# PPWangyc/video-spike

Hardware: AMD Instinct MI355X
Metric: clips/sec (16-frame 224x224) train step (higher is better)
Workload: dtype bf16; 1 GPU; C2 ViT-Tiny/16 16x224x224 -> 128 neurons, encoder+head fwd+bwd+AdamW; model=vmae_tiny, global_batch=128, clips_per_gpu=128, seq_len=1568, parallelism=dp1

## Files before the change

include/vspike.h:

```cpp
#ifndef VSPIKE_H
#define VSPIKE_H

#include <stddef.h>
#include <stdint.h>

#ifdef __cplusplus
extern "C" {
#endif

#define VS_OK 0
#define VS_EINVAL (-1)

#define VS_F32 0
#define VS_BF16 1
#define VS_U8 2
#define VS_F64 4
#define VS_FP8 3

int vs_version(void);
const char* vs_build_id(void);
const char* vs_last_error(void);
int vs_device_arch(char* buf, int n);
int vs_struct_size(int which);

// ... 308 lines not shown
#define VS_PATH_GEMM_FULLK    7
#define VS_PATH_GEMM_RING     8
#define VS_PATH_GEMM_TILE     9
#define VS_PATH_GEMM_F32     10
#define VS_PATH_GEMM_LN_FWD  11
#define VS_PATH_GEMM_LN_BWD  12
#define VS_PATH_ATTN_FWD     13
#define VS_PATH_ATTN_BWD     14
#define VS_PATH_ATTN_F32     15
#define VS_PATH_PATCH_FUSED  16
#define VS_PATH_DW_GROUPED   17
#define VS_PATH_MLP_FWD      18
#define VS_PATH_MLP_BWD      19
#define VS_PATH_GEMM_FP8     20
#define VS_PATH_PATCH_DW     21
#define VS_PATH_CONV_IGEMM   22
#define VS_PATH_CONV_DW      23
#define VS_PATH_GEMM_G256    24
#define VS_PATH_GEMM_DW256   25
#define VS_PATH_TOKEN_POOL   26
#define VS_PATH_CLS_EMBED    27
#define VS_PATH_EMBED_HEAD   28
#define VS_PATH_INFO_NCE     29
#define VS_PATH_COUNT        30
int vs_dispatch_counts(int64_t* out, int n);
int vs_dispatch_reset(void);
#define VS_LN_KERNELS 9
int vs_ln_dispatch_counts(int64_t* out, int n);
#define VS_RRR_PATH_WIDE   0
#define VS_RRR_PATH_SMOOTH 1
#define VS_RRR_PATH_COUNT  2
int vs_rrr_dispatch_counts(int64_t* out, int n);
int vs_g256_scratch_free(void);

#define VS_KNOB_DW_OLD       0
#define VS_KNOB_NO_SKINNY    1
#define VS_KNOB_NO_SLAB      2
#define VS_KNOB_NO_BIG       3
#define VS_KNOB_NO_WRES      4
#define VS_KNOB_WRES_GBWD    5
#define VS_KNOB_NO_WSLAB     6
#define VS_KNOB_WSLAB        7
#define VS_KNOB_WSLAB_G      8
#define VS_KNOB_PANEL        9
#define VS_KNOB_NO_PANEL    10
#define VS_KNOB_PANEL_GRID  11
#define VS_KNOB_NO_FULLK    12
#define VS_KNOB_NO_RING     13
#define VS_KNOB_NO_LNF_FUSE 14
#define VS_KNOB_NO_LN_FUSE  15
#define VS_KNOB_DW_BM       16
#define VS_KNOB_DW_BN       17
#define VS_KNOB_DW_SPLITS   18
#define VS_KNOB_DW_STAGES   19
#define VS_KNOB_LN_BLOCKS   20
#define VS_KNOB_DH_F32      21
#define VS_KNOB_NO_PATCH_FUSED 22
#define VS_KNOB_NO_DW_GROUP 23
#define VS_KNOB_ATTN_VARIANT 24
#define VS_KNOB_SLAB_WV     25
#define VS_KNOB_WRES_WV     26
#define VS_KNOB_WRES_DBG    27
#define VS_KNOB_G256        28
#define VS_KNOB_G256_GRID   29
#define VS_KNOB_G256_DBG    30
#define VS_KNOB_NO_DW256    31
#define VS_KNOB_G256_STAGGER 32
#define VS_KNOB_CONV_DW128  33
#define VS_KNOB_CONV_MFMA   34
#define VS_KNOB_DW256_ALL   36
#define VS_KNOB_LN_FWD_BLOCKS 37
#define VS_KNOB_G256_A3     35
#define VS_KNOB_COUNT       40
int vs_knob_get(int knob);
int vs_knob_set(int knob, int value);
int vs_knob_default(int knob);
int vs_debug_knobs(void);

#ifdef __cplusplus
}
#endif
#endif
```

video-spike_amd/csrc/gemm.hip:

```cpp
#include <cstdlib>

#include "common.h"
#include "gemm_common.h"
#include "gemm_dw.h"

namespace vs {

template <int BM, int BN, int TM, int TN, uint32_t EF, int PARTS = 1>
__device__ __forceinline__ void store_tile(const EpiParams& e, float* lds, const f32x4 (&acc)[TM][TN], int64_t m0,
                                           int64_t n0, int split) {
  static_assert(PARTS == 1 || (PARTS == 2 && BM / 2 == BM / 2 / 16 * 16), "row halves");
  const bool first_split = split == 0;
  const uint32_t F = epi_flags<EF>(e);
  constexpr int LDT = BN + 4;
  constexpr int WM = BM / 2, WN = BN / 2, RB = BM / PARTS;
  const int tid = threadIdx.x, lane = tid & 63, wid = tid >> 6, wr = wid >> 1, wc = wid & 1;
  constexpr int CPR = BN / 8;
  constexpr int RPP = 256 / CPR;
  const int cg = tid % CPR;
  const int64_t n = n0 + cg * 8;
  const bool vec = e.vec_ok && n + 8 <= e.N;
  float bias8[8];
  if ((F & VS_EPI_BIAS) && vec && !(F & VS_EPI_ATOMIC) && !e.part) ld8(e.bias, n, 0, bias8);
#pragma unroll
  for (int part = 0; part < PARTS; ++part) {
    const int64_t mp = m0 + part * RB;
    __syncthreads();
    if (PARTS == 1 || wr == part) {
#pragma unroll
      for (int i = 0; i < TM; ++i)
#pragma unroll
        for (int j = 0; j < TN; ++j)
// ... 517 lines not shown
  VS_GMARK(4);
#ifdef VS_STAMP
  if ((threadIdx.x & 63) == 0) {
    const int w_ = blockIdx.x * 4 + (threadIdx.x >> 6);
    if (w_ < 8192) {
      g_gstamp[8 * w_ + 5] = __builtin_amdgcn_s_getreg((31 << 11) | 4);
      g_gstamp[8 * w_ + 6] = __builtin_amdgcn_s_memrealtime();
    }
  }
#endif
}

struct LnBwdParams {
  const float* x;
  int64_t ldx;
  const float* mean;
  const float* rstd;
  const float* gamma;
  const float* dres;
  int64_t ldr;
  float* dx;
  int64_t lddx;
  bf16_t* dx_lp;
  float* part;
  const float* beta;
  float eps;
  bf16_t* h;
  int64_t ldh;
  float* mean_out;
  float* rstd_out;
};

template <int NT, bool BKC, uint32_t EF, bool LNB = false, bool LNF = false, int WV = 4>
__global__ __launch_bounds__(64 * WV, 2) __attribute__((amdgpu_waves_per_eu(WV / 2, WV / 2))) void gemm_bf16_slab_kernel(const bf16_t* __restrict__ A, int64_t lda,
                                                                const bf16_t* __restrict__ B, int64_t ldb, int64_t K,
                                                                EpiParams e, LnBwdParams ln) {
  constexpr int RT = 16 * WV, NTH = 64 * WV, PR = NTH / 16;
  using OA = OperandBf16<RT, true>;
  using OB = OperandBf16<64, BKC>;
  constexpr int N = 64 * NT, TM = 2, TN = NT * 2, WN = N / 2;
  constexpr int STAGE = OA::BYTES + NT * OB::BYTES;
  constexpr int LDT = N + 4;
  static_assert(64 * LDT * 4 <= 2 * STAGE, "epilogue staging (64 rows at a time) fits the ring");
  static_assert(WV == 4 || WV == 8, "4 or 8 waves");
  __shared__ __attribute__((aligned(16))) char smem[2 * STAGE];

  const int tid = threadIdx.x, lane = tid & 63, wid = tid >> 6, wr = wid >> 1, wc = wid & 1;
  const int64_t G = gridDim.x;
  const int64_t r_begin = (int64_t)blockIdx.x * e.M / G, r_end = ((int64_t)blockIdx.x + 1) * e.M / G;
  const int nk = (int)(K / 64);
  const int gl = tid & 15, rsub = tid >> 4;
  float4 pg[NT], pb[NT];
#pragma unroll
  for (int j = 0; j < NT; ++j) {
    pg[j] = make_float4(0.f, 0.f, 0.f, 0.f);
    pb[j] = make_float4(0.f, 0.f, 0.f, 0.f);
  }

  for (int64_t m0 = r_begin; m0 < r_end; m0 += RT) {
    const int64_t m_end = m0 + RT < r_end ? m0 + RT : r_end;
    f32x4 acc[TM][TN];
#pragma unroll
    for (int i = 0; i < TM; ++i)
#pragma unroll
      for (int j = 0; j < TN; ++j) acc[i][j] = f32x4{0.f, 0.f, 0.f, 0.f};
    auto issue = [&](int t, char* st) {
      const int64_t k0 = (int64_t)t * 64;
// ... 219 lines not shown
  }
  if constexpr (LNB) {
    float* red = (float*)smem;
    __syncthreads();
#pragma unroll
    for (int j = 0; j < NT; ++j) {
#define VS_RED(V)                               \
  {                                             \
    _Pragma("unroll") for (int o = 16; o < 64; o <<= 1) { \
      V.x += __shfl_xor(V.x, o, 64);            \
      V.y += __shfl_xor(V.y, o, 64);            \
      V.z += __shfl_xor(V.z, o, 64);            \
      V.w += __shfl_xor(V.w, o, 64);            \
    }                                           \
  }
      VS_RED(pg[j]) VS_RED(pb[j])
#undef VS_RED
      if (lane < 16) {
        *(float4*)&red[(0 * WV + wid) * N + 4 * (gl + 16 * j)] = pg[j];
        *(float4*)&red[(1 * WV + wid) * N + 4 * (gl + 16 * j)] = pb[j];
      }
    }
    __syncthreads();
    for (int c = tid; c < N; c += NTH) {
      float a = (red[0 * N + c] + red[1 * N + c]) + (red[2 * N + c] + red[3 * N + c]);
      float b = (red[WV * N + c] + red[(WV + 1) * N + c]) + (red[(WV + 2) * N + c] + red[(WV + 3) * N + c]);
      if constexpr (WV == 8) {
        a += (red[4 * N + c] + red[5 * N + c]) + (red[6 * N + c] + red[7 * N + c]);
        b += (red[12 * N + c] + red[13 * N + c]) + (red[14 * N + c] + red[15 * N + c]);
      }
      ln.part[(int64_t)blockIdx.x * 2 * N + c] = a;
      ln.part[(int64_t)blockIdx.x * 2 * N + N + c] = b;
    }
  }
}

struct PatchGeo {
  int F, C, H, W;
  int n_tok, HpWp, Wp;
};

template <int NT, bool COLS>
__global__ __launch_bounds__(256, 2) void patch_embed_fwd_kernel(const float* __restrict__ px, PatchGeo g,
                                                                 const bf16_t* __restrict__ B, int64_t K,
                                                                 EpiParams e, bf16_t* __restrict__ cols) {
  using OA = OperandBf16<64, true>;
  using OB = OperandBf16<64, true>;
  constexpr int N = 64 * NT, TM = 2, TN = NT * 2, WN = N / 2, NR = 3;
  constexpr int STAGE = OA::BYTES + NT * OB::BYTES;
  constexpr int LDT = N + 4;
  static_assert(64 * LDT * 4 <= 2 * STAGE, "epilogue staging fits the ring");
  __shared__ __attribute__((aligned(16))) char smem[2 * STAGE];

  const int tid = threadIdx.x, lane = tid & 63, wid = tid >> 6, wr = wid >> 1, wc = wid & 1;
  const int64_t G = gridDim.x;
  const int64_t r_begin = (int64_t)blockIdx.x * e.M / G, r_end = ((int64_t)blockIdx.x + 1) * e.M / G;
  const int nk = (int)(K / 64);
  const int ii = (tid >> 2) & 3, jq = tid & 3;
  const int64_t plane = (int64_t)g.H * g.W;

  for (int64_t m0 = r_begin; m0 < r_end; m0 += 64) {
    const int64_t m_end = m0 + 64 < r_end ? m0 + 64 : r_end;
    int64_t base[4];
#pragma unroll
    for (int s = 0; s < 4; ++s) {
      int64_t m = m0 + (tid >> 4) + 16 * s;
// ... 1338 lines not shown
}

template <int BM, int BN, uint32_t EF>
static void launch_bf16_ring_ef(const vs_gemm_desc* d, unsigned nblk, const GridMap& g, const EpiParams& e,
                                hipStream_t s) {
  const bf16_t* a = (const bf16_t*)d->a;
  const bf16_t* b = (const bf16_t*)d->b;
  if (d->a_kcontig && d->b_kcontig)
    hipLaunchKernelGGL((gemm_bf16_ring_kernel<BM, BN, true, true, EF>), dim3(nblk), dim3(256), 0, s, a, d->lda, b, d->ldb, d->K, g, e);
  else if (d->a_kcontig)
    hipLaunchKernelGGL((gemm_bf16_ring_kernel<BM, BN, true, false, EF>), dim3(nblk), dim3(256), 0, s, a, d->lda, b, d->ldb, d->K, g, e);
  else if (d->b_kcontig)
    hipLaunchKernelGGL((gemm_bf16_ring_kernel<BM, BN, false, true, EF>), dim3(nblk), dim3(256), 0, s, a, d->lda, b, d->ldb, d->K, g, e);
  else
    hipLaunchKernelGGL((gemm_bf16_ring_kernel<BM, BN, false, false, EF>), dim3(nblk), dim3(256), 0, s, a, d->lda, b, d->ldb, d->K, g, e);
}

template <int KT, uint32_t EF>
static void launch_bf16_panel_ef(const vs_gemm_desc* d, unsigned grid, int64_t items, const EpiParams& e,
                                 hipStream_t s) {
  const bf16_t* a = (const bf16_t*)d->a;
  const bf16_t* b = (const bf16_t*)d->b;
  if (d->b_kcontig)
    hipLaunchKernelGGL((gemm_bf16_panel_kernel<KT, true, EF>), dim3(grid), dim3(256), 0, s, a, d->lda, b, d->ldb, items, e);
  else
    hipLaunchKernelGGL((gemm_bf16_panel_kernel<KT, false, EF>), dim3(grid), dim3(256), 0, s, a, d->lda, b, d->ldb, items, e);
}

static inline bool slab_wide(int64_t M, int64_t K, unsigned grid) {
  const int f = knob(VS_KNOB_SLAB_WV);
  if (f == 4 || f == 8) return f == 8;
  return M / (int64_t)grid >= 256 && K >= 384;
}
template <int NT, uint32_t EF, bool LNB = false, bool LNF = false>
static void launch_bf16_slab_ef(const vs_gemm_desc* d, unsigned grid, const EpiParams& e, hipStream_t s,
                                const LnBwdParams& ln = LnBwdParams{}) {
  const bf16_t* a = (const bf16_t*)d->a;
  const bf16_t* b = (const bf16_t*)d->b;
  if (slab_wide(d->M, d->K, grid)) {
    if (d->b_kcontig)
      hipLaunchKernelGGL((gemm_bf16_slab_kernel<NT, true, EF, LNB, LNF, 8>), dim3(grid), dim3(512), 0, s, a, d->lda, b,
                         d->ldb, d->K, e, ln);
    else
      hipLaunchKernelGGL((gemm_bf16_slab_kernel<NT, false, EF, LNB, LNF, 8>), dim3(grid), dim3(512), 0, s, a, d->lda, b,
                         d->ldb, d->K, e, ln);
    return;
  }
  if (d->b_kcontig)
    hipLaunchKernelGGL((gemm_bf16_slab_kernel<NT, true, EF, LNB, LNF>), dim3(grid), dim3(256), 0, s, a, d->lda, b,
                       d->ldb, d->K, e, ln);
  else
    hipLaunchKernelGGL((gemm_bf16_slab_kernel<NT, false, EF, LNB, LNF>), dim3(grid), dim3(256), 0, s, a, d->lda, b,
                       d->ldb, d->K, e, ln);
}
template <int NT>
static void launch_bf16_slab(const vs_gemm_desc* d, unsigned grid, const EpiParams& e, hipStream_t s) {
  switch (e.flags) {
    case 0: launch_bf16_slab_ef<NT, 0u>(d, grid, e, s); break;
    case VS_EPI_BIAS: launch_bf16_slab_ef<NT, (uint32_t)VS_EPI_BIAS>(d, grid, e, s); break;
    case VS_EPI_BIAS | VS_EPI_POS:
      launch_bf16_slab_ef<NT, (uint32_t)(VS_EPI_BIAS | VS_EPI_POS)>(d, grid, e, s);
      break;
    default: launch_bf16_slab_ef<NT, (uint32_t)(VS_EPI_BIAS | VS_EPI_RESIDUAL)>(d, grid, e, s); break;
  }
}

template <int KT, uint32_t EF>
static void launch_bf16_wslab_ef(const vs_gemm_desc* d, unsigned grid, const EpiParams& e, hipStream_t s) {
  const bf16_t* a = (const bf16_t*)d->a;
  const bf16_t* b = (const bf16_t*)d->b;
  if (d->b_kcontig)
// ... 70 lines not shown
template <bool BKC, bool P8>
static int g256_no_scratch_all() {
  int ok = 1;
#define CHK_(EF)                                                                                    \
  {                                                                                                 \
    hipFuncAttributes fa{};                                                                          \
    if (hipFuncGetAttributes(&fa, (const void*)gemm_bf16_g256_kernel<BKC, P8, EF>) != hipSuccess || \
        fa.localSizeBytes != 0)                                                                     \
      ok = 0;                                                                                       \
  }
  CHK_(0u) CHK_((uint32_t)VS_EPI_BIAS) CHK_((uint32_t)(VS_EPI_BIAS | VS_EPI_RESIDUAL))
  CHK_((uint32_t)(VS_EPI_BIAS | VS_EPI_GELU)) CHK_((uint32_t)VS_EPI_GELU_BWD)
  CHK_((uint32_t)(VS_EPI_BIAS | VS_EPI_GELU | VS_EPI_GELU_GRAD)) CHK_((uint32_t)VS_EPI_MUL_AUX)
#undef CHK_
  return ok;
}

#define VS_EPI_SWITCH(F, CALL)                                                             \
  switch (F) {                                                                             \
    case 0: CALL(0u); break;                                                               \
    case VS_EPI_BIAS: CALL((uint32_t)VS_EPI_BIAS); break;                                  \
    case VS_EPI_BIAS | VS_EPI_RESIDUAL: CALL((uint32_t)(VS_EPI_BIAS | VS_EPI_RESIDUAL)); break; \
    case VS_EPI_BIAS | VS_EPI_GELU: CALL((uint32_t)(VS_EPI_BIAS | VS_EPI_GELU)); break;    \
    case VS_EPI_GELU_BWD: CALL((uint32_t)VS_EPI_GELU_BWD); break;                          \
    case VS_EPI_BIAS | VS_EPI_GELU | VS_EPI_GELU_GRAD:                                     \
      CALL((uint32_t)(VS_EPI_BIAS | VS_EPI_GELU | VS_EPI_GELU_GRAD)); break;               \
    case VS_EPI_MUL_AUX: CALL((uint32_t)VS_EPI_MUL_AUX); break;                            \
    default: CALL(kEpiRuntime); break;                                                     \
  }

extern "C" int vs_g256_scratch_free(void) {
  return g256_no_scratch_all<true, true>() & g256_no_scratch_all<false, true>() & g256_no_scratch_all<false, false>();
}

static void launch_bf16_g256(const vs_gemm_desc* d, const G256Map& g, unsigned grid, const EpiParams& e,
                             hipStream_t s) {
#define L_(EF) launch_bf16_g256_ef<EF>(d, g, grid, e, s)
  VS_EPI_SWITCH(e.flags, L_)
#undef L_
}

static void launch_bf16_big(const vs_gemm_desc* d, unsigned nblk, const GridMap& g, const EpiParams& e, hipStream_t s) {
#define L_(EF) launch_bf16_big_ef<EF>(d, nblk, g, e, s)
  VS_EPI_SWITCH(e.flags, L_)
#undef L_
}

template <int BM, int BN>
static void launch_bf16(const vs_gemm_desc* d, unsigned nblk, const GridMap& g, const EpiParams& e, hipStream_t s) {
#define L_(EF) launch_bf16_ef<BM, BN, EF>(d, nblk, g, e, s)
  VS_EPI_SWITCH(e.flags, L_)
#undef L_
}

template <int BM, int BN>
static void launch_bf16_ring(const vs_gemm_desc* d, unsigned nblk, const GridMap& g, const EpiParams& e, hipStream_t s) {
#define L_(EF) launch_bf16_ring_ef<BM, BN, EF>(d, nblk, g, e, s)
  VS_EPI_SWITCH(e.flags, L_)
#undef L_
}

template <int KT>
static void launch_bf16_panel(const vs_gemm_desc* d, unsigned grid, int64_t items, const EpiParams& e, hipStream_t s) {
#define L_(EF) launch_bf16_panel_ef<KT, EF>(d, grid, items, e, s)
  VS_EPI_SWITCH(e.flags, L_)
#undef L_
// ... 619 lines not shown
```

video-spike_amd/csrc/runtime.hip:

```cpp
#include <atomic>
#include <cstdlib>
#include <mutex>
#include <string.h>
#include <vector>

#include "common.h"

#ifndef VS_BUILD_ID
#define VS_BUILD_ID "unknown"
#endif

namespace vs {

static thread_local char g_err[512] = "";
thread_local int g_timer_tag = -1;

void set_error(const char* msg) {
  strncpy(g_err, msg, sizeof(g_err) - 1);
  g_err[sizeof(g_err) - 1] = 0;
}

struct KnobDef {
  const char* env;
  int dflt;
};
static const KnobDef kKnobs[VS_KNOB_COUNT] = {
    {"VSPIKE_DW_OLD", 0},      {"VSPIKE_NO_SKINNY", 0},    {"VSPIKE_NO_SLAB", 0},      {"VSPIKE_NO_BIG", 0},
    {"VSPIKE_NO_WRES", 0},     {"VSPIKE_WRES_GBWD", 0},    {"VSPIKE_NO_WSLAB", 0},     {"VSPIKE_WSLAB", 0},
    {"VSPIKE_WSLAB_G", 512},   {"VSPIKE_PANEL", 0},        {"VSPIKE_NO_PANEL", 0},     {"VSPIKE_PANEL_GRID", 512},
    {"VSPIKE_NO_FULLK", 0},    {"VSPIKE_NO_RING", 0},      {"VSPIKE_NO_LNF_FUSE", 0},  {"VSPIKE_NO_LN_FUSE", 0},
    {"VSPIKE_DW_BM", 0},       {"VSPIKE_DW_BN", 0},        {"VSPIKE_DW_SPLITS", 0},    {"VSPIKE_DW_STAGES", 0},
    {"VSPIKE_LN_BLOCKS", 0},   {"VSPIKE_DH_F32", 0},       {"VSPIKE_NO_PATCH_FUSED", 0}, {"VSPIKE_NO_DW_GROUP", 0},
    {"VSPIKE_ATTN_VARIANT", 0}, {"VSPIKE_SLAB_WV", 0}, {"VSPIKE_WRES_WV", 0}, {"VSPIKE_WRES_DBG", 0}, {"VSPIKE_G256", 0}, {"VSPIKE_G256_GRID", 0}, {"VSPIKE_G256_DBG", 0}, {"VSPIKE_NO_DW256", 0}, {"VSPIKE_G256_STAGGER", 0}, {"VSPIKE_CONV_DW128", 0},
    {"VSPIKE_CONV_MFMA", 0}, {"VSPIKE_G256_A3", 0}, {"VSPIKE_DW256_ALL", 0}, {"VSPIKE_LN_FWD_BLOCKS", 0},
    {nullptr, 0}};
static std::atomic<int> g_knob[VS_KNOB_COUNT];
static std::once_flag g_knob_once;
static void knob_init() {
  for (int i = 0; i < VS_KNOB_COUNT; ++i) {
    int v = kKnobs[i].dflt;
    if (kKnobs[i].env) {
      const char* e = getenv(kKnobs[i].env);
      if (e && e[0]) v = (int)strtol(e, nullptr, 0);
    }
    g_knob[i].store(v, std::memory_order_relaxed);
  }
}
int knob(int id) {
  std::call_once(g_knob_once, knob_init);
  return g_knob[id].load(std::memory_order_relaxed);
}

static std::atomic<int64_t> g_dispatch[VS_PATH_COUNT];
void count_path(int id) { g_dispatch[id].fetch_add(1, std::memory_order_relaxed); }
static std::atomic<int64_t> g_rrr_dispatch[VS_RRR_PATH_COUNT];
void count_rrr(int id) { g_rrr_dispatch[id].fetch_add(1, std::memory_order_relaxed); }
static std::atomic<int64_t> g_ln_dispatch[2 * VS_LN_KERNELS];
void count_ln(int kernel, bool bwd) {
  g_ln_dispatch[(bwd ? VS_LN_KERNELS : 0) + kernel].fetch_add(1, std::memory_order_relaxed);
}

struct TimerState {
  std::mutex mu;
  unsigned mask = 0;
  std::vector<hipEvent_t> pool;
  std::vector<std::pair<hipEvent_t, hipEvent_t>> pairs[VS_TIMER_COUNT];
  double bytes[VS_TIMER_COUNT] = {};
  hipEvent_t get() {
// ... 139 lines not shown
```

video-spike_amd/vspike/_lib.py:

```python
from __future__ import annotations

import ctypes
import os

import torch

from .build import LIB_PATH

VS_F32, VS_BF16, VS_U8, VS_FP8, VS_F64 = 0, 1, 2, 3, 4
EPI_BIAS, EPI_GELU, EPI_RELU, EPI_RESIDUAL, EPI_POS = 0x1, 0x2, 0x4, 0x8, 0x10
EPI_GELU_BWD, EPI_RELU_BWD, EPI_ATOMIC, EPI_ACCUM = 0x20, 0x40, 0x80, 0x100
EPI_GELU_GRAD, EPI_MUL_AUX = 0x200, 0x400
BWD_DEFER_JOIN = 0x1
BWD_DEFER_LAST = 0x2
BWD_FUSE_LN = 0x4
TIMER_ATTN_FWD, TIMER_ATTN_BWD, TIMER_GEMM, TIMER_GEMM_DW, TIMER_LN_FWD, TIMER_LN_BWD, TIMER_ADAMW, TIMER_MISC = range(8)
TIMER_NAMES = ("attn_fwd", "attn_bwd", "gemm", "gemm_dw", "ln_fwd", "ln_bwd", "adamw", "misc",
               "fwd_qkv", "fwd_proj", "fwd_fc1", "fwd_fc2", "dx_fc2", "dx_fc1", "dx_proj", "dx_qkv",
               "dw_fc2", "dw_fc1", "dw_proj", "dw_qkv",
               "fwd_mlp", "dx_mlp",
               "fp8_quant",
               "conv_fwd", "conv_dx", "conv_dw", "bn")

PATH_NAMES = ("gemm_dw", "gemm_skinny", "gemm_slab", "gemm_big", "gemm_wres", "gemm_wslab", "gemm_panel",
              "gemm_fullk", "gemm_ring", "gemm_tile", "gemm_f32", "gemm_ln_fwd", "gemm_ln_bwd", "attn_fwd",
              "attn_bwd", "attn_f32", "patch_fused", "dw_grouped", "mlp_fwd", "mlp_bwd", "gemm_fp8", "patch_dw",
              "conv_igemm", "conv_dw", "gemm_g256", "gemm_dw256", "token_pool")
PATH_COUNT = 27
CONTRAST_PATH_NAMES = ("cls_embed", "embed_head", "info_nce")
EXTRA_PATH_NAMES = CONTRAST_PATH_NAMES
KNOB_NAMES = ("dw_old", "no_skinny", "no_slab", "no_big", "no_wres", "wres_gbwd", "no_wslab", "wslab", "wslab_g",
              "panel", "no_panel", "panel_grid", "no_fullk", "no_ring", "no_lnf_fuse", "no_ln_fuse", "dw_bm", "dw_bn",
              "dw_splits", "dw_stages", "ln_blocks", "dh_f32", "no_patch_fused", "no_dw_group", "attn_variant", "slab_wv", "wres_wv", "wres_dbg",
              "g256", "g256_grid", "g256_dbg", "no_dw256", "g256_stagger", "conv_dw128", "conv_mfma", "g256_a3", "dw256_all", "ln_fwd_blocks")
KNOB_COUNT = 40

c_i32, c_i64, c_u32, c_f32, c_p, c_sz = (ctypes.c_int32, ctypes.c_int64, ctypes.c_uint32, ctypes.c_float,
                                         ctypes.c_void_p, ctypes.c_size_t)
c_f64 = ctypes.c_double


class VsError(RuntimeError):
    pass


class GemmDesc(ctypes.Structure):
    _fields_ = [("dtype", c_i32), ("out_dtype", c_i32), ("a_kcontig", c_i32), ("b_kcontig", c_i32),
                ("M", c_i64), ("N", c_i64), ("K", c_i64),
                ("a", c_p), ("lda", c_i64), ("b", c_p), ("ldb", c_i64), ("c", c_p), ("ldc", c_i64),
                ("epilogue", c_u32), ("alpha", c_f32), ("bias", c_p),
                ("residual", c_p), ("ld_residual", c_i64), ("pos", c_p), ("pos_rows", c_i64),
                ("aux_in", c_p), ("ld_aux_in", c_i64), ("aux_out", c_p), ("ld_aux_out", c_i64),
                ("split_k", c_i32), ("reserved", c_i32), ("a_rowsum", c_p), ("workspace", c_p),
                ("workspace_bytes", c_i64)]


class Conv3dDesc(ctypes.Structure):
    _fields_ = [("N", c_i64), ("Di", c_i64), ("Hi", c_i64), ("Wi", c_i64), ("Ci", c_i64),
                ("Do", c_i64), ("Ho", c_i64), ("Wo", c_i64), ("Co", c_i64),
                ("kd", c_i32), ("kh", c_i32), ("kw", c_i32), ("sd", c_i32), ("sh", c_i32), ("sw", c_i32),
                ("pd", c_i32), ("ph", c_i32), ("pw", c_i32), ("reserved", c_i32)]


class VitLayer(ctypes.Structure):
    _fields_ = [("dtype", c_i32), ("heads", c_i32), ("batch", c_i64), ("tokens", c_i64), ("hidden", c_i64),
                ("mlp", c_i64), ("ln_eps", c_f32), ("attn_scale", c_f32),
                ("ln1_g", c_p), ("ln1_b", c_p), ("ln2_g", c_p), ("ln2_b", c_p),
                ("w_qkv", c_p), ("b_qkv", c_p), ("w_proj", c_p), ("b_proj", c_p),
                ("w_fc1", c_p), ("b_fc1", c_p), ("w_fc2", c_p), ("b_fc2", c_p),
                ("x_in", c_p), ("h1", c_p), ("mean1", c_p), ("rstd1", c_p), ("qkv", c_p), ("attn_o", c_p),
                ("lse", c_p), ("y", c_p), ("h2", c_p), ("mean2", c_p), ("rstd2", c_p), ("a_pre", c_p),
                ("a_act", c_p), ("x_out", c_p), ("fp8_ws", c_p), ("fp8_ws_bytes", c_i64),
                ("next_ln_g", c_p), ("next_ln_b", c_p), ("next_h1", c_p), ("next_mean1", c_p), ("next_rstd1", c_p),
                ("ln1_ready", c_i32), ("reserved7", c_i32)]


class VitLayerGrad(ctypes.Structure):
    _fields_ = [("ln1_g", c_p), ("ln1_b", c_p), ("ln2_g", c_p), ("ln2_b", c_p),
                ("w_qkv", c_p), ("b_qkv", c_p), ("w_proj", c_p), ("b_proj", c_p),
                ("w_fc1", c_p), ("b_fc1", c_p), ("w_fc2", c_p), ("b_fc2", c_p),
                ("dx_out", c_p), ("dx_out_lp", c_p), ("dx_in", c_p), ("dx_in_lp", c_p),
                ("d_a", c_p), ("d_h", c_p), ("dy", c_p), ("dy_lp", c_p), ("d_o", c_p), ("d_qkv", c_p),
                ("attn_ws", c_p), ("ln_ws", c_p), ("gemm_ws", c_p), ("gemm_ws_bytes", c_i64),
                ("flags", c_i32), ("reserved", c_i32), ("chain", c_p)]


PROTOTYPES = {
    "vs_version": (ctypes.c_int, []),
    "vs_build_id": (ctypes.c_char_p, []),
    "vs_dispatch_counts": (ctypes.c_int, [ctypes.POINTER(c_i64), ctypes.c_int]),
    "vs_dispatch_reset": (ctypes.c_int, []),
    "vs_ln_dispatch_counts": (ctypes.c_int, [ctypes.POINTER(c_i64), ctypes.c_int]),
    "vs_g256_scratch_free": (ctypes.c_int, []),
    "vs_knob_get": (ctypes.c_int, [ctypes.c_int]),
    "vs_knob_set": (ctypes.c_int, [ctypes.c_int, ctypes.c_int]),
    "vs_knob_default": (ctypes.c_int, [ctypes.c_int]),
    "vs_debug_knobs": (ctypes.c_int, []),
    "vs_mse_loss": (ctypes.c_int, [c_i64, c_p, c_p, c_p, c_p, c_f32, c_p, c_p]),
    "vs_comm_unique_id": (ctypes.c_int, [c_p]),
    "vs_comm_init": (ctypes.c_int, [ctypes.POINTER(c_p), c_p, c_i32, c_i32]),
    "vs_comm_allreduce_bucket": (ctypes.c_int, [c_p, c_p, c_i64, c_i32, c_p]),
    "vs_comm_finalize": (ctypes.c_int, [c_p]),
    "vs_mse_loss_bwd": (ctypes.c_int, [c_i64, c_p, c_p, c_p, c_p, c_p]),
    "vs_last_error": (ctypes.c_char_p, []),
    "vs_device_arch": (ctypes.c_int, [ctypes.c_char_p, ctypes.c_int]),
    "vs_struct_size": (ctypes.c_int, [ctypes.c_int]),
    "vs_gemm": (ctypes.c_int, [ctypes.POINTER(GemmDesc), c_p]),
    "vs_layernorm_fwd": (ctypes.c_int, [c_i32, c_i64, c_i64, c_p, c_i64, c_p, c_p, c_f32, c_p, c_i64, c_p, c_p,
                                        c_p]),
    "vs_layernorm_bwd_workspace_bytes": (c_sz, [c_i64, c_i64]),
    "vs_gemm_splitk_workspace_bytes": (c_sz, [c_i32, c_i64, c_i64, c_i64]),
    "vs_video_preprocess": (ctypes.c_int, [c_i32, c_i64, c_i64, c_i64, c_i64, c_p, ctypes.POINTER(c_i32), c_i32,
                                           c_i64, ctypes.POINTER(c_f32), ctypes.POINTER(c_f32), c_p, c_p]),
    "vs_layernorm_bwd": (ctypes.c_int, [c_i64, c_i64, c_p, c_i64, c_p, c_i64, c_p, c_p, c_p, c_p, c_i64, c_p,
                                        c_i64, c_p, c_p, c_p, c_p, c_p]),
    "vs_layernorm_bwd_dt": (ctypes.c_int, [ctypes.c_int32, c_i64, c_i64, c_p, c_i64, c_p, c_i64, c_p, c_p, c_p, c_p, c_i64, c_p,
                                        c_i64, c_p, c_p, c_p, c_p, c_p]),
    "vs_gemm_ln_fwd": (ctypes.c_int, [ctypes.POINTER(GemmDesc), c_p, c_p, ctypes.c_float, c_p, c_i64, c_p, c_p, c_p]),
    "vs_gemm_ln_bwd": (ctypes.c_int, [ctypes.POINTER(GemmDesc), c_p, c_i64, c_p, c_p, c_p, c_p, c_i64, c_p, c_i64,
                                      c_p, c_p, c_p, c_p, c_p]),
    "vs_mlp_fused_ok": (ctypes.c_int, [c_i64, c_i64, c_i64]),
    "vs_mlp_fwd_ln": (ctypes.c_int, [c_i64, c_i64, c_i64, c_p, c_i64, c_p, c_p, c_p, c_p, c_p, c_i64, c_p, c_i64,
                                     c_p, c_p, c_f32, c_p, c_i64, c_p, c_p, c_p]),
    "vs_quant_mxfp8": (ctypes.c_int, [c_i32, c_i64, c_i64, c_p, c_i64, c_p, c_i64, c_p, c_i64, c_p]),
    "vs_gemm_mxfp8": (ctypes.c_int, [ctypes.POINTER(GemmDesc), c_p, c_i64, c_p, c_i64, c_p]),
    "vs_mlp_fwd": (ctypes.c_int, [c_i64, c_i64, c_i64, c_p, c_i64, c_p, c_p, c_p, c_p, c_p, c_i64, c_p, c_i64, c_p]),
# ... 233 lines not shown
```

Baseline: 4183 clips/sec.

## Add persistent triple-buffered slab GEMM kernel with fused LayerNorm backward

Adds a persistent 512-thread slab GEMM kernel with fused LayerNorm backward. It keeps three LDS stages and prefetches the next slab's first K tiles while the current slab's LN-backward epilogue runs, so slab boundaries no longer drain the load pipeline. The kernel is only used when a new knob is set to 1 (default 0) and K/64 is a multiple of 3, with grid size defaulting to the CU count. Separately, the existing slab kernel's waves-per-EU hint is fixed at 2 instead of WV/2, which changes register allocation and occupancy for the 8-wave variant on the default path. Occupancy and launch-count query helpers are also exported.

```diff
diff --git a/include/vspike.h b/include/vspike.h
--- a/include/vspike.h
+++ b/include/vspike.h
@@ -364,6 +364,9 @@
 #define VS_RRR_PATH_COUNT  2
 int vs_rrr_dispatch_counts(int64_t* out, int n);
 int vs_g256_scratch_free(void);
+int vs_slab_occupancy(int nt, int bkc, int lnb, int wv, int pipe);
+int vs_slab_pipe_grid(int slabs);
+int64_t vs_slab_pipe_launches(void);
 
 #define VS_KNOB_DW_OLD       0
 #define VS_KNOB_NO_SKINNY    1
@@ -403,6 +406,8 @@
 #define VS_KNOB_DW256_ALL   36
 #define VS_KNOB_LN_FWD_BLOCKS 37
 #define VS_KNOB_G256_A3     35
+#define VS_KNOB_SLAB_PIPE   38
+#define VS_KNOB_SLAB_PIPE_GRID 39
 #define VS_KNOB_COUNT       40
 int vs_knob_get(int knob);
 int vs_knob_set(int knob, int value);
diff --git a/video-spike_amd/csrc/gemm.hip b/video-spike_amd/csrc/gemm.hip
--- a/video-spike_amd/csrc/gemm.hip
+++ b/video-spike_amd/csrc/gemm.hip
@@ -1,3 +1,4 @@
+#include <atomic>
 #include <cstdlib>
 
 #include "common.h"
@@ -581,7 +582,7 @@
 };
 
 template <int NT, bool BKC, uint32_t EF, bool LNB = false, bool LNF = false, int WV = 4>
-__global__ __launch_bounds__(64 * WV, 2) __attribute__((amdgpu_waves_per_eu(WV / 2, WV / 2))) void gemm_bf16_slab_kernel(const bf16_t* __restrict__ A, int64_t lda,
+__global__ __launch_bounds__(64 * WV, 2) __attribute__((amdgpu_waves_per_eu(2, 2))) void gemm_bf16_slab_kernel(const bf16_t* __restrict__ A, int64_t lda,
                                                                 const bf16_t* __restrict__ B, int64_t ldb, int64_t K,
                                                                 EpiParams e, LnBwdParams ln) {
   constexpr int RT = 16 * WV, NTH = 64 * WV, PR = NTH / 16;
@@ -867,6 +868,249 @@
       ln.part[(int64_t)blockIdx.x * 2 * N + c] = a;
       ln.part[(int64_t)blockIdx.x * 2 * N + N + c] = b;
     }
+  }
+}
+
+template <int NT, bool BKC>
+__global__ __launch_bounds__(512, 1) void gemm_bf16_slab_pipe_kernel(const bf16_t* __restrict__ A, int64_t lda,
+                                                                     const bf16_t* __restrict__ B, int64_t ldb, int64_t K,
+                                                                     int G, EpiParams e, LnBwdParams ln) {
+  constexpr int WV = 8, RT = 128, NTH = 512, PR = 32;
+  using OA = OperandBf16<RT, true>;
+  using OB = OperandBf16<64, BKC>;
+  constexpr int N = 64 * NT, TM = 2, TN = NT * 2, WN = N / 2;
+  constexpr int STAGE = OA::BYTES + NT * OB::BYTES;
+  constexpr int LDT = N + 4;
+  constexpr int STG = PR * LDT * 4;
+  constexpr int PER = OA::PIECES / WV + NT * (OB::PIECES / WV);
+  static_assert(STG + 2 * WV * N * 4 <= STAGE, "staging and the slab-end reduction share one stage");
+  static_assert(RT / PR == 4 && NTH / 16 == PR, "one LN' pass per wave row");
+  __shared__ __attribute__((aligned(16))) char st0[STAGE];
+  __shared__ __attribute__((aligned(16))) char st1[STAGE];
+  __shared__ __attribute__((aligned(16))) char st2[STAGE];
+
+  const int tid = threadIdx.x, lane = tid & 63, wid = tid >> 6, wr = wid >> 1, wc = wid & 1;
+  const int nk = (int)(K / 64);
+  const int gl = tid & 15, rsub = tid >> 4;
+  float* stg = (float*)st2;
+  float* red = (float*)(st2 + STG);
+  float4 pg[NT], pb[NT];
+#pragma unroll
+  for (int j = 0; j < NT; ++j) {
+    pg[j] = make_float4(0.f, 0.f, 0.f, 0.f);
+    pb[j] = make_float4(0.f, 0.f, 0.f, 0.f);
+  }
+  auto raw_sync = [&]() {
+    asm volatile("s_waitcnt lgkmcnt(0)" ::: "memory");
+    __builtin_amdgcn_s_barrier();
+    asm volatile("" ::: "memory");
+  };
+  auto late = [](int64_t v) {
+    uint32_t lo = __builtin_amdgcn_readfirstlane((uint32_t)v), hi = __builtin_amdgcn_readfirstlane((uint32_t)((uint64_t)v >> 32));
+    asm volatile("" : "+s"(lo), "+s"(hi));
+    return (int64_t)(((uint64_t)hi << 32) | lo);
+  };
+  auto issue = [&](int64_t m0, int64_t m_end, int t, char* st) {
+    const int64_t k0 = (int64_t)t * 64;
+    int ln_ = lane;
+    asm volatile("" : "+v"(ln_));
+    OA::template dma_nw<WV>(st, A, lda, m0, m_end, k0, wid, ln_);
+#pragma unroll
+    for (int j = 0; j < NT; ++j) OB::template dma_nw<WV>(st + OA::BYTES + j * OB::BYTES, B, ldb, j * 64, N, k0, wid, ln_);
+  };
+  struct RowOps {
+    float4 xv[NT], rv[NT];
+    float mu, rs;
+  };
+  auto row_load = [&](RowOps& o, int64_t mq, int64_t m_end) {
+    int rsub = tid >> 4, gl = tid & 15;
+    asm volatile("" : "+v"(rsub), "+v"(gl));
+    int64_t m = mq + rsub;
+    m = m < m_end ? m : m_end - 1;
+#pragma unroll
+    for (int j = 0; j < NT; ++j) {
+      const int c = 4 * (gl + 16 * j);
+      o.xv[j] = *(const float4*)(ln.x + m * ln.ldx + c);
+      o.rv[j] = ln.dres ? *(const float4*)(ln.dres + m * ln.ldr + c) : make_float4(0.f, 0.f, 0.f, 0.f);
+    }
+    o.mu = ln.mean[m];
+    o.rs = ln.rstd[m];
+  };
+
+  int g = (int)blockIdx.x;
+  int64_t r_end = ((int64_t)g + 1) * e.M / G;
+  int64_t m0 = (int64_t)g * e.M / G;
+  issue(m0, m0 + RT < r_end ? m0 + RT : r_end, 0, st0);
+  issue(m0, m0 + RT < r_end ? m0 + RT : r_end, 1, st1);
+  for (;;) {
+    const int64_t m_end = m0 + RT < r_end ? m0 + RT : r_end;
+    const bool slab_done = m_end == r_end;
+    const int g_nx = slab_done ? g + (int)gridDim.x : g;
+    const bool more = g_nx < G;
+    const int64_t m0_nx = slab_done ? (int64_t)g_nx * e.M / G : m0 + RT;
+    const int64_t r_end_nx = slab_done ? ((int64_t)g_nx + 1) * e.M / G : r_end;
+    const int64_t m_end_nx = m0_nx + RT < r_end_nx ? m0_nx + RT : r_end_nx;
+    const bool mine = (int64_t)wr * 32 < m_end - m0;
+
+    f32x4 acc[TM][TN];
+#pragma unroll
+    for (int i = 0; i < TM; ++i)
+#pragma unroll
+      for (int j = 0; j < TN; ++j) acc[i][j] = f32x4{0.f, 0.f, 0.f, 0.f};
+    RowOps ops[2];
+    auto compute = [&](const char* sa) {
+#pragma unroll
+      for (int kk = 0; kk < 2; ++kk) {
+        bf16x8 af[TM], bfr[TN];
+#pragma unroll
+        for (int i = 0; i < TM; ++i) af[i] = OA::frag(sa, wr * 32 + i * 16, kk, lane);
+#pragma unroll
+        for (int j = 0; j < TN; ++j) {
+          const int col = wc * WN + j * 16;
+          bfr[j] = OB::frag(sa + OA::BYTES + (col >> 6) * OB::BYTES, col & 63, kk, lane);
+        }
+#pragma unroll
+        for (int i = 0; i < TM; ++i)
+#pragma unroll
+          for (int j = 0; j < TN; ++j) acc[i][j] = __builtin_amdgcn_mfma_f32_16x16x32_bf16(af[i], bfr[j], acc[i][j], 0, 0, 0);
+      }
+    };
+    auto step = [&](int t, auto sc, auto lastc) {
+      constexpr int S = decltype(sc)::value;
+      constexpr bool LAST = decltype(lastc)::value != 0;
+      const char* cur = S == 0 ? st0 : (S == 1 ? st1 : st2);
+      char* far = S == 0 ? st2 : (S == 1 ? st0 : st1);
+      if (!LAST || S < 2 || more) asm volatile("s_waitcnt vmcnt(%0)" ::"n"(PER) : "memory");
+      else asm volatile("s_waitcnt vmcnt(0)" ::: "memory");
+      asm volatile("s_waitcnt lgkmcnt(0)" ::: "memory");
+      __builtin_amdgcn_s_barrier();
+      asm volatile("" ::: "memory");
+      if constexpr (!LAST || S == 0) {
+        issue(m0, m_end, t + 2, far);
+      } else {
+        if (more) issue(late(m0_nx), late(m_end_nx), S - 1, far);
+        if constexpr (S == 2) row_load(ops[0], late(m0), late(m_end));
+      }
+      if (mine) compute(cur);
+    };
+    for (int t = 0; t < nk - 3; t += 3) {
+      step(t, IC<0>{}, IC<0>{});
+      step(t + 1, IC<1>{}, IC<0>{});
+      step(t + 2, IC<2>{}, IC<0>{});
+    }
+    step(nk - 3, IC<0>{}, IC<1>{});
+    step(nk - 2, IC<1>{}, IC<1>{});
+    step(nk - 1, IC<2>{}, IC<1>{});
+#pragma unroll
+    for (int q = 0; q < RT / PR; ++q) {
+      if (m0 + q * PR >= m_end) break;
+      raw_sync();
+      const int64_t mq = late(m0 + q * PR);
+      if (wr == q) {
+#pragma unroll
+        for (int i = 0; i < TM; ++i)
+#pragma unroll
+          for (int j = 0; j < TN; ++j)
+#pragma unroll
+            for (int r = 0; r < 4; ++r)
+              stg[(i * 16 + (lane >> 4) * 4 + r) * LDT + wc * WN + j * 16 + (lane & 15)] = acc[i][j][r] * e.alpha;
+      }
+      if (q + 1 < RT / PR && mq + PR < m_end) row_load(ops[(q + 1) & 1], mq + PR, m_end);
+      float4 gam[NT];
+      {
+        int gl = tid & 15;
+        asm volatile("" : "+v"(gl));
+#pragma unroll
+        for (int j = 0; j < NT; ++j) gam[j] = *(const float4*)(ln.gamma + 4 * (gl + 16 * j));
+      }
+      raw_sync();
+      constexpr float inv = 1.f / (float)N;
+      int rsub = tid >> 4, gl = tid & 15;
+      asm volatile("" : "+v"(rsub), "+v"(gl));
+      RowOps& o_ = ops[q & 1];
+      const int64_t m = mq + rsub;
+      const bool valid = m < m_end;
+      float4 d[NT];
+      float s1 = 0.f, s2 = 0.f;
+#pragma unroll
+      for (int j = 0; j < NT; ++j) {
+        d[j] = *(const float4*)(stg + rsub * LDT + 4 * (gl + 16 * j));
+#define VS_LNB(C)                                  \
+  {                                                \
+    const float xh = (o_.xv[j].C - o_.mu) * o_.rs; \
+    const float gy = d[j].C * gam[j].C;            \
+    if (valid) {                                   \
+      pg[j].C += d[j].C * xh;                      \
+      pb[j].C += d[j].C;                           \
+    }                                              \
+    o_.xv[j].C = xh;                               \
+    d[j].C = gy;                                   \
+    s1 += gy;                                      \
+    s2 += gy * xh;                                 \
+  }
+        VS_LNB(x) VS_LNB(y) VS_LNB(z) VS_LNB(w)
+#undef VS_LNB
+      }
+#pragma unroll
+      for (int o = 8; o > 0; o >>= 1) {
+        s1 += __shfl_xor(s1, o, 64);
+        s2 += __shfl_xor(s2, o, 64);
+      }
+      const float m1 = s1 * inv, m2 = s2 * inv;
+      if (valid) {
+#pragma unroll
+        for (int j = 0; j < NT; ++j) {
+          const int c = 4 * (gl + 16 * j);
+          float4 o;
+          o.x = o_.rs * (d[j].x - m1 - o_.xv[j].x * m2) + o_.rv[j].x;
+          o.y = o_.rs * (d[j].y - m1 - o_.xv[j].y * m2) + o_.rv[j].y;
+          o.z = o_.rs * (d[j].z - m1 - o_.xv[j].z * m2) + o_.rv[j].z;
+          o.w = o_.rs * (d[j].w - m1 - o_.xv[j].w * m2) + o_.rv[j].w;
+          *(float4*)(ln.dx + m * ln.lddx + c) = o;
+          if (ln.dx_lp) {
+            uint2 u;
+            u.x = (uint32_t)f2bf(o.x) | ((uint32_t)f2bf(o.y) << 16);
+            u.y = (uint32_t)f2bf(o.z) | ((uint32_t)f2bf(o.w) << 16);
+            *(uint2*)(ln.dx_lp + m * ln.lddx + c) = u;
+          }
+        }
+      }
+    }
+    if (slab_done) {
+#pragma unroll
+      for (int j = 0; j < NT; ++j) {
+#define VS_RED(V)                               \
+  {                                             \
+    _Pragma("unroll") for (int o = 16; o < 64; o <<= 1) { \
+      V.x += __shfl_xor(V.x, o, 64);            \
+      V.y += __shfl_xor(V.y, o, 64);            \
+      V.z += __shfl_xor(V.z, o, 64);            \
+      V.w += __shfl_xor(V.w, o, 64);            \
+    }                                           \
+  }
+        VS_RED(pg[j]) VS_RED(pb[j])
+#undef VS_RED
+        if (lane < 16) {
+          *(float4*)&red[(0 * WV + wid) * N + 4 * (gl + 16 * j)] = pg[j];
+          *(float4*)&red[(1 * WV + wid) * N + 4 * (gl + 16 * j)] = pb[j];
+        }
+        pg[j] = make_float4(0.f, 0.f, 0.f, 0.f);
+        pb[j] = make_float4(0.f, 0.f, 0.f, 0.f);
+      }
+      raw_sync();
+      for (int c = tid; c < N; c += NTH) {
+        float a = (red[0 * N + c] + red[1 * N + c]) + (red[2 * N + c] + red[3 * N + c]);
+        float b = (red[WV * N + c] + red[(WV + 1) * N + c]) + (red[(WV + 2) * N + c] + red[(WV + 3) * N + c]);
+        a += (red[4 * N + c] + red[5 * N + c]) + (red[6 * N + c] + red[7 * N + c]);
+        b += (red[12 * N + c] + red[13 * N + c]) + (red[14 * N + c] + red[15 * N + c]);
+        ln.part[(int64_t)g * 2 * N + c] = a;
+        ln.part[(int64_t)g * 2 * N + N + c] = b;
+      }
+    }
+    if (!more) break;
+    g = g_nx;
+    m0 = m0_nx;
+    r_end = r_end_nx;
   }
 }
 
@@ -2271,11 +2515,39 @@
   if (f == 4 || f == 8) return f == 8;
   return M / (int64_t)grid >= 256 && K >= 384;
 }
+static int device_cus() {
+  static const int cus = [] {
+    int dev = 0, n = 256;
+    if (hipGetDevice(&dev) == hipSuccess) (void)hipDeviceGetAttribute(&n, hipDeviceAttributeMultiprocessorCount, dev);
+    return n > 0 ? n : 256;
+  }();
+  return cus;
+}
+static unsigned slab_pipe_grid(unsigned G) {
+  const int f = knob(VS_KNOB_SLAB_PIPE_GRID);
+  const unsigned p = f > 0 ? (unsigned)f : (unsigned)device_cus();
+  return p < G ? p : G;
+}
+static inline bool slab_pipe(int64_t K) { return knob(VS_KNOB_SLAB_PIPE) == 1 && (K / 64) % 3 == 0; }
+static std::atomic<int64_t> g_slab_pipe_launches{0};
 template <int NT, uint32_t EF, bool LNB = false, bool LNF = false>
 static void launch_bf16_slab_ef(const vs_gemm_desc* d, unsigned grid, const EpiParams& e, hipStream_t s,
                                 const LnBwdParams& ln = LnBwdParams{}) {
   const bf16_t* a = (const bf16_t*)d->a;
   const bf16_t* b = (const bf16_t*)d->b;
+  if constexpr (LNB) {
+    if (slab_wide(d->M, d->K, grid) && slab_pipe(d->K)) {
+      const unsigned p = slab_pipe_grid(grid);
+      g_slab_pipe_launches.fetch_add(1, std::memory_order_relaxed);
+      if (d->b_kcontig)
+        hipLaunchKernelGGL((gemm_bf16_slab_pipe_kernel<NT, true>), dim3(p), dim3(512), 0, s, a, d->lda, b, d->ldb, d->K,
+                           (int)grid, e, ln);
+      else
+        hipLaunchKernelGGL((gemm_bf16_slab_pipe_kernel<NT, false>), dim3(p), dim3(512), 0, s, a, d->lda, b, d->ldb, d->K,
+                           (int)grid, e, ln);
+      return;
+    }
+  }
   if (slab_wide(d->M, d->K, grid)) {
     if (d->b_kcontig)
       hipLaunchKernelGGL((gemm_bf16_slab_kernel<NT, true, EF, LNB, LNF, 8>), dim3(grid), dim3(512), 0, s, a, d->lda, b,
@@ -2412,6 +2684,32 @@
 extern "C" int vs_g256_scratch_free(void) {
   return g256_no_scratch_all<true, true>() & g256_no_scratch_all<false, true>() & g256_no_scratch_all<false, false>();
 }
+
+template <int NT, bool BKC>
+static int slab_occupancy_nt(int lnb, int wv, int pipe) {
+  int n = -1;
+  hipError_t r = hipErrorInvalidValue;
+  if (pipe) r = hipOccupancyMaxActiveBlocksPerMultiprocessor(&n, gemm_bf16_slab_pipe_kernel<NT, BKC>, 512, 0);
+  else if (lnb && wv == 8) r = hipOccupancyMaxActiveBlocksPerMultiprocessor(&n, gemm_bf16_slab_kernel<NT, BKC, 0u, true, false, 8>, 512, 0);
+  else if (lnb && wv == 4) r = hipOccupancyMaxActiveBlocksPerMultiprocessor(&n, gemm_bf16_slab_kernel<NT, BKC, 0u, true, false, 4>, 256, 0);
+  else if (wv == 8) r = hipOccupancyMaxActiveBlocksPerMultiprocessor(&n, gemm_bf16_slab_kernel<NT, BKC, 0u, false, false, 8>, 512, 0);
+  else if (wv == 4) r = hipOccupancyMaxActiveBlocksPerMultiprocessor(&n, gemm_bf16_slab_kernel<NT, BKC, 0u, false, false, 4>, 256, 0);
+  return r == hipSuccess ? n : -1;
+}
+extern "C" int vs_slab_occupancy(int nt, int bkc, int lnb, int wv, int pipe) {
+  if (pipe && !(lnb && wv == 8)) return -1;
+  switch (nt * 2 + (bkc ? 1 : 0)) {
+    case 2: return slab_occupancy_nt<1, false>(lnb, wv, pipe);
+    case 3: return slab_occupancy_nt<1, true>(lnb, wv, pipe);
+    case 4: return slab_occupancy_nt<2, false>(lnb, wv, pipe);
+    case 5: return slab_occupancy_nt<2, true>(lnb, wv, pipe);
+    case 6: return slab_occupancy_nt<3, false>(lnb, wv, pipe);
+    case 7: return slab_occupancy_nt<3, true>(lnb, wv, pipe);
+    default: return -1;
+  }
+}
+extern "C" int64_t vs_slab_pipe_launches(void) { return g_slab_pipe_launches.load(std::memory_order_relaxed); }
+extern "C" int vs_slab_pipe_grid(int slabs) { return slabs > 0 ? (int)slab_pipe_grid((unsigned)slabs) : 0; }
 
 static void launch_bf16_g256(const vs_gemm_desc* d, const G256Map& g, unsigned grid, const EpiParams& e,
                              hipStream_t s) {
diff --git a/video-spike_amd/csrc/runtime.hip b/video-spike_amd/csrc/runtime.hip
--- a/video-spike_amd/csrc/runtime.hip
+++ b/video-spike_amd/csrc/runtime.hip
@@ -33,7 +33,7 @@
     {"VSPIKE_LN_BLOCKS", 0},   {"VSPIKE_DH_F32", 0},       {"VSPIKE_NO_PATCH_FUSED", 0}, {"VSPIKE_NO_DW_GROUP", 0},
     {"VSPIKE_ATTN_VARIANT", 0}, {"VSPIKE_SLAB_WV", 0}, {"VSPIKE_WRES_WV", 0}, {"VSPIKE_WRES_DBG", 0}, {"VSPIKE_G256", 0}, {"VSPIKE_G256_GRID", 0}, {"VSPIKE_G256_DBG", 0}, {"VSPIKE_NO_DW256", 0}, {"VSPIKE_G256_STAGGER", 0}, {"VSPIKE_CONV_DW128", 0},
     {"VSPIKE_CONV_MFMA", 0}, {"VSPIKE_G256_A3", 0}, {"VSPIKE_DW256_ALL", 0}, {"VSPIKE_LN_FWD_BLOCKS", 0},
-    {nullptr, 0}};
+    {"VSPIKE_SLAB_PIPE", 0}, {"VSPIKE_SLAB_PIPE_GRID", 0}};
 static std::atomic<int> g_knob[VS_KNOB_COUNT];
 static std::once_flag g_knob_once;
 static void knob_init() {
diff --git a/video-spike_amd/vspike/_lib.py b/video-spike_amd/vspike/_lib.py
--- a/video-spike_amd/vspike/_lib.py
+++ b/video-spike_amd/vspike/_lib.py
@@ -32,7 +32,8 @@
 KNOB_NAMES = ("dw_old", "no_skinny", "no_slab", "no_big", "no_wres", "wres_gbwd", "no_wslab", "wslab", "wslab_g",
               "panel", "no_panel", "panel_grid", "no_fullk", "no_ring", "no_lnf_fuse", "no_ln_fuse", "dw_bm", "dw_bn",
               "dw_splits", "dw_stages", "ln_blocks", "dh_f32", "no_patch_fused", "no_dw_group", "attn_variant", "slab_wv", "wres_wv", "wres_dbg",
-              "g256", "g256_grid", "g256_dbg", "no_dw256", "g256_stagger", "conv_dw128", "conv_mfma", "g256_a3", "dw256_all", "ln_fwd_blocks")
+              "g256", "g256_grid", "g256_dbg", "no_dw256", "g256_stagger", "conv_dw128", "conv_mfma", "g256_a3", "dw256_all", "ln_fwd_blocks",
+              "slab_pipe", "slab_pipe_grid")
 KNOB_COUNT = 40
 
 c_i32, c_i64, c_u32, c_f32, c_p, c_sz = (ctypes.c_int32, ctypes.c_int64, ctypes.c_uint32, ctypes.c_float,
@@ -92,6 +93,9 @@
     "vs_dispatch_reset": (ctypes.c_int, []),
     "vs_ln_dispatch_counts": (ctypes.c_int, [ctypes.POINTER(c_i64), ctypes.c_int]),
     "vs_g256_scratch_free": (ctypes.c_int, []),
+    "vs_slab_occupancy": (ctypes.c_int, [ctypes.c_int] * 5),
+    "vs_slab_pipe_grid": (ctypes.c_int, [ctypes.c_int]),
+    "vs_slab_pipe_launches": (c_i64, []),
     "vs_knob_get": (ctypes.c_int, [ctypes.c_int]),
     "vs_knob_set": (ctypes.c_int, [ctypes.c_int, ctypes.c_int]),
     "vs_knob_default": (ctypes.c_int, [ctypes.c_int]),
```

Result: no change. 4155 clips/sec (-0.7%).
